# walkernr/neuralMelting

Measured on AMD Instinct MI355X. Metric: MC sweeps/sec (whole node), LJ 4^3 cells, 8x8 PxT grid, higher is better.
Workload: dtype f64

## Files before the change

### include/nm.h

```cpp
#ifndef NM_H
#define NM_H
#include <stdint.h>

#ifdef __cplusplus
extern "C" {
#endif

#define NM_OK 0
#define NM_ERR_ARG (-1)
#define NM_ERR_HIP (-2)
#define NM_ERR_STATE (-3)
#define NM_ERR_UNSUPPORTED (-4)

#define NM_EL_LJ 0
#define NM_EL_AL 1
#define NM_EL_NI 2
#define NM_EL_CU 3

#define NM_THERMO_COLS 17
#define NM_TRACE_COLS 4
#define NM_STATS_COLS 10

typedef struct nm_ctx nm_ctx;

typedef struct nm_config {
    int32_t size;
    int32_t element;
    int32_t natoms;
    int32_t np, nt;
    int32_t row0, nrows;
    int32_t nstps;
    int32_t bulk;
    int32_t iter_revert;
    int32_t device;
    uint32_t seed;
    double ppos, pvol;
// ... 75 lines not shown
```

### neuralmelting_amd/_lib.py

```python
import ctypes as C
import os

_HERE = os.path.dirname(os.path.abspath(__file__))
LIB_PATH = os.environ.get('NM_HIP_LIB') or os.path.join(_HERE, 'libnm_hip.so')

c_double_p = C.POINTER(C.c_double)
c_float_p = C.POINTER(C.c_float)
c_int_p = C.POINTER(C.c_int)
c_uint64_p = C.POINTER(C.c_uint64)
c_int32_p = C.POINTER(C.c_int32)

NM_OK, NM_ERR_ARG, NM_ERR_HIP, NM_ERR_STATE, NM_ERR_UNSUPPORTED = 0, -1, -2, -3, -4
NM_EL_LJ, NM_EL_AL, NM_EL_NI, NM_EL_CU = 0, 1, 2, 3
NM_THERMO_COLS, NM_TRACE_COLS, NM_STATS_COLS = 17, 4, 10

SYMBOLS = ('nm_create', 'nm_destroy', 'nm_last_error', 'nm_create_note', 'nm_nslots', 'nm_natoms', 'nm_cus_per_replica', 'nm_heal_count', 'nm_get_const',
           'nm_get_slots', 'nm_set_slots', 'nm_snapshot', 'nm_snapshot_fetch', 'nm_run_cycles_recorded', 'nm_record_capacity', 'nm_snapshot_pending',
           'nm_set_state', 'nm_get_state', 'nm_init_lattice', 'nm_lattice_state', 'nm_set_thermo', 'nm_set_step', 'nm_run_md', 'nm_run_block', 'nm_run_cycles', 'nm_get_thermo', 'nm_adapt',
           'nm_exchange', 'nm_synchronize', 'nm_get_status', 'nm_format_thrm', 'nm_format_traj', 'nm_append_outputs', 'nm_timing_reset', 'nm_timing_get', 'nm_stats_get', 'nm_eval',
           'nm_set_rng_tape', 'nm_set_exchange_tape', 'nm_set_trace', 'nm_get_trace', 'nm_get_perm', 'nm_set_counters',
           'nm_get_exchange_crit')


DISTR_SYMBOLS = ('nm_distr_histograms', 'nm_distr_angles', 'nm_distr_sfactor', 'nm_distr_bondorder', 'nm_distr_last_error')
PARSE_SYMBOLS = ('nm_parse_thrm', 'nm_parse_traj', 'nm_parse_last_error')


class NMConfig(C.Structure):
    _fields_ = [('size', C.c_int32), ('element', C.c_int32), ('natoms', C.c_int32), ('np', C.c_int32),
# ... 90 lines not shown
```

### neuralmelting_amd/csrc/nm_api.hip

```cpp
#include "../../include/nm.h"
#include "nm_kernels.h"
#include "nm_distr.h"
#include "nm_format.h"
#include "nm_parse.h"
#include "nm_lattice.h"
#include "../../include/nm_distr.h"
#include "../../include/nm_parse.h"

#include <algorithm>
#include <cmath>
#include <cstdio>
#include <cstdlib>
#include <cstring>
#include <deque>
#include <string>
#include <thread>
#include <type_traits>
#include <vector>

using namespace nm;

namespace {

typedef Cfg<512, 4, 256, 192, unsigned char, true, true, 0, 128, true, true> CfgSmallQ2;
// ... 65 lines not shown
static_assert(CfgMidSC::RHO_LDS && CfgMidSCQ4::RHO_LDS && !CfgLargeSC::RHO_LDS, "densities: in LDS at 864 atoms, in the spill at 2048");

thread_local std::string g_create_error;

struct EvPair { hipEvent_t a, b; bool used; uint32_t launch_id; };

}

struct nm_ctx {
    nm_config cfg;
    int N, nslots, slot0, kind;
    int cus;
    bool whole_rows;
    double *d_xbuf;
    uint32_t launch_id;
    double lat, mass, kB, mvv2e, ftm2v, nktv2p, skin, rc;
    int pot;
    double sc_eps, sc_a2, sc_c;
    uint32_t step;
    hipStream_t stream;
    double *d_x, *d_v, *d_box, *d_steps, *d_therm, *d_count, *d_et, *d_pf, *d_tq, *d_stats;
    float *d_ratio;
    int *d_slot2buf, *d_status, *d_status_acc, *d_halt, *d_rerun, *d_nswaps, *d_order;
    unsigned long long *d_last_ticks;
    bool use_order;
    unsigned int *d_census;
    unsigned int census_base = 0, census_cbase = 0;
    unsigned int *d_rowsync = nullptr;
    bool over;
    struct Op { int kind, arg, trace; uint32_t step, launch_id; int rec = -1, rec0 = 0; };
// ... 59 lines not shown
    p.kB = c->kB; p.mvv2e = c->mvv2e; p.ftm2v = c->ftm2v; p.nktv2p = c->nktv2p;
    p.rc = c->rc; p.skin = c->skin;
    p.sc_eps = c->sc_eps; p.sc_a2 = c->sc_a2; p.sc_c = c->sc_c;
    p.x = c->d_x; p.v = c->d_v; p.box = c->d_box; p.steps = c->d_steps; p.therm = c->d_therm;
    p.count = c->d_count; p.ratio = c->d_ratio; p.slot2buf = c->d_slot2buf;
    p.et = c->d_et; p.pf = c->d_pf; p.tq = c->d_tq;
    p.status = c->d_status; p.stats = c->d_stats;
    p.tape = c->d_tape; p.tape_off = c->d_tape_off;
    p.nbr_g = c->d_nbr; p.aux_g = c->d_aux;
    p.prof = c->d_prof;
    p.cus = c->cus; p.xbuf = c->d_xbuf; p.launch_id = c->launch_id;
    p.census = c->cus > 1 ? c->d_census : nullptr; p.over = (c->cus > 1 && c->over) ? 1 : 0;
    p.census_base = c->census_base; p.census_cbase = c->census_cbase;
    p.plain_granules = 1;
    if (const char *e = std::getenv("NM_PLAIN_GRANULES")) p.plain_granules = std::atoi(e);
    p.dbg = 0;
    p.tline = c->d_tline;
    if (const char *e = std::getenv("NM_DBG")) p.dbg = std::atoi(e);
    p.inj_rebuild = -1; p.inj_q = 0;
    const char *e = testing() ? std::getenv("NM_INJECT_OVERFLOW") : nullptr;
    if (e) {
        int n = -1, q = 0;
        if (std::sscanf(e, "%d,%d", &n, &q) >= 1) { p.inj_rebuild = n; p.inj_q = q; }
    }
    p.status_acc = c->d_status_acc; p.halt = c->d_halt; p.rerun_mask = nullptr; p.inj_census = 0;
    p.order = (c->use_order && (c->cus == 1 || c->over)) ? c->d_order : nullptr; p.last_ticks = c->d_last_ticks;
}

unsigned int nm_grid(int nslots, int q) { return q == 1 ? (unsigned int)nslots : (unsigned int)(8 * q * ((nslots + 7) / 8)); }
size_t census_words(int nslots) { return 1 + (size_t)8 * ((nslots + 7) / 8); }
// ... 486 lines not shown

    nm_ctx *c = new nm_ctx();
    c->cfg = *cfg;
    c->h_P.assign(cfg->P, cfg->P + cfg->np); c->h_T.assign(cfg->T, cfg->T + cfg->nt);
    c->cfg.P = c->h_P.data(); c->cfg.T = c->h_T.data();
    c->N = cfg->natoms;
    c->nslots = by_slots ? cfg->nslots : cfg->nrows * cfg->nt;
    c->slot0 = by_slots ? cfg->slot0 : cfg->row0 * cfg->nt;
    c->whole_rows = (c->slot0 % cfg->nt == 0) && (c->nslots % cfg->nt == 0);
    c->cfg.row0 = c->slot0 / cfg->nt;
    c->cfg.nrows = c->whole_rows ? c->nslots / cfg->nt : 0;
    c->step = 0;
    c->trace_on = 0; c->trace_mod = 0; c->trace_cap = 0; c->xtape_n = 0;
    c->ev_next = 0; c->launches = 0; c->total_ms = 0.0;
    c->skin = cfg->natoms <= 512 ? 0.4 : cfg->natoms <= 1024 ? 0.55 : 0.6;
    if (const char *e = std::getenv("NM_SKIN")) { const double v = std::atof(e); if (v > 0.0 && v < 1.0) c->skin = v; }
    c->lat = 1.122; c->mass = 1.0; c->kB = 1.0; c->mvv2e = 1.0; c->ftm2v = 1.0; c->nktv2p = 1.0;
    c->rc = 2.5; c->pot = 0; c->sc_eps = 0.0; c->sc_a2 = 0.0; c->sc_c = 0.0;
    if (const lat::ScElement *s = lat::sc_element(cfg->element)) {
        c->lat = s->lat; c->mass = s->mass; c->kB = 8.617343e-5; c->mvv2e = 1.0364269e-4; c->ftm2v = 1.0 / 1.0364269e-4;
        c->nktv2p = 1.6021765e6; c->rc = s->rc; c->skin = s->skin; c->pot = s->pot;
        c->sc_eps = s->eps; c->sc_a2 = s->a * s->a; c->sc_c = s->c;
        if (cfg->element == NM_EL_AL)
            if (const char *e = std::getenv("NM_SKIN_AL")) { const double v = std::atof(e); if (v > 0.0 && v < 3.0) c->skin = v; }
    }

    c->h_et.resize(c->nslots); c->h_pf.resize(c->nslots); c->h_tq.resize(c->nslots);
    for (int k = 0; k < c->nslots; ++k) {
        const int i = (c->slot0 + k) / cfg->nt, j = (c->slot0 + k) % cfg->nt;
        const double Pi = (double)cfg->P[i], Tj = (double)cfg->T[j];
// ... 1072 lines not shown
```

### neuralmelting_amd/csrc/nm_device.h

```cpp
#pragma once
#include <hip/hip_runtime.h>
#include <stdint.h>

namespace nm {

enum : uint32_t { S_ROLL = 0, S_ACC = 1, S_VOL = 2, S_DISP_XY = 3, S_DISP_Z = 4, S_VEL_A = 5, S_VEL_B = 6,
                  S_EXCH = 7, S_ITER_XY = 8, S_ITER_Z = 9, S_ITER_ACC = 10 };

enum : int { ST_LIST_OVERFLOW = 1, ST_BOX_TOO_SMALL = 2, ST_TAPE_EXHAUSTED = 4, ST_NONFINITE = 8, ST_SYNC_TIMEOUT = 16, ST_NOT_RESIDENT = 32,
             ST_FORCE_RANGE = 64 };

struct KParams {
    int N, nslots, slot0;
    int mod, nstps, bulk, iter_revert;
    int eval_only;
    int md_mode;
    uint32_t seed, step;
    double ppos, pvol, lat, mass;
    double kB, mvv2e, ftm2v, nktv2p;
    double rc, skin;
    double sc_eps, sc_a2, sc_c;
    double *x, *v, *box, *steps, *therm;
    double *count;
    float *ratio;
// ... 19 lines not shown
    unsigned int census_base, census_cbase;
    int *status_acc;
    int *halt;
    const int *rerun_mask;
    int inj_census;
    int over;
    const int *order;
    unsigned long long *last_ticks;
    int ncycles, nt, row0;
    unsigned int *rowbar, *rowgo;
    int *cyc_abort;
    int *nswaps;
    double *xcrit;
    double *rec;
    uint32_t rec_tag0;
};

enum : int { NM_REC_HEAD = 19, NM_REC_BOX = 17, NM_REC_TAG = 18 };

__device__ __forceinline__ void report_status(const KParams &p, int slot, int bits, bool stops)
{
    if (!bits) return;
    atomicOr(&p.status[slot], bits);
    if (p.status_acc) atomicOr(&p.status_acc[slot], bits);
    if (stops && p.halt) atomicCAS(p.halt, 0, (int)p.launch_id);
}
__device__ __forceinline__ bool halted(const KParams &p)
{
    if (!p.halt) return false;
    const int h = __hip_atomic_load(p.halt, __ATOMIC_RELAXED, __HIP_MEMORY_SCOPE_AGENT);
// ... 162 lines not shown
```

### neuralmelting_amd/csrc/nm_kernels.h

```cpp
#pragma once
#include "nm_device.h"
#include "nm_math.h"

namespace nm {

constexpr int NVMAX = 16;

#if defined(NM_PROF) || defined(NM_EXPERIMENT)
#define NM_DBG(bit) (p.dbg & (bit))
#else
#define NM_DBG(bit) false
#endif
#ifdef NM_EXPERIMENT
#define TL_EVALS 512
#define TLINE(k) do { if (tl && tl_n < TL_EVALS && (tid & 63) == 0) tl[((size_t)(q * NW + (tid >> 6)) * TL_EVALS + tl_n) * 8 + (k)] = wall_clock64(); } while (0)
#define TLINE_PREV(k) do { if (tl && tl_n > 0 && tl_n <= TL_EVALS && (tid & 63) == 0) tl[((size_t)(q * NW + (tid >> 6)) * TL_EVALS + tl_n - 1) * 8 + (k)] = wall_clock64(); } while (0)
#ifdef NM_TL_REBUILD
#define RTL(k) do { if (tl && tl_n < TL_EVALS && (tid & 63) == 0) tl[((size_t)(q * NW + (tid >> 6)) * TL_EVALS + tl_n) * 8 + (k)] = wall_clock64(); } while (0)
#undef TLINE
#undef TLINE_PREV
#define TLINE(k) do { if ((k) < 3 && tl && tl_n < TL_EVALS && (tid & 63) == 0) tl[((size_t)(q * NW + (tid >> 6)) * TL_EVALS + tl_n) * 8 + (k)] = wall_clock64(); } while (0)
#define TLINE_PREV(k) do { } while (0)
#else
#define RTL(k) do { } while (0)
#endif
#else
#define TLINE(k) do { } while (0)
#define TLINE_PREV(k) do { } while (0)
#define RTL(k) do { } while (0)
#endif
#ifdef NM_PROF
#define NM_PROF_SLOTS 16
#define PROF_DECL unsigned long long prof_acc[NM_PROF_SLOTS] = {}; unsigned long long prof_t0 = 0;
#define PROF_BEGIN() do { __builtin_amdgcn_sched_barrier(0); prof_t0 = __builtin_readcyclecounter(); __builtin_amdgcn_sched_barrier(0); } while (0)
#define PROF_END(k) do { __builtin_amdgcn_sched_barrier(0); prof_acc[k] += __builtin_readcyclecounter() - prof_t0; __builtin_amdgcn_sched_barrier(0); } while (0)
#else
#define PROF_DECL
#define PROF_BEGIN() do { } while (0)
#define PROF_END(k) do { } while (0)
#endif

extern __shared__ __align__(16) unsigned char nm_lds[];

template <typename T, size_t OFF>
// ... 64 lines not shown
    static constexpr size_t OFF_CNTS = OFF_X0S + (LDS_LIST2 ? A3 : 0);
    static constexpr size_t LDS_NATURAL = OFF_CNTS + (LDS_LIST2 ? pad8((size_t)NMAX * sizeof(unsigned short)) : 0);
    static constexpr size_t LDS_BYTES = LDS_NATURAL > (size_t)82 * 1024 ? LDS_NATURAL : (size_t)82 * 1024;
    static constexpr size_t AUX_SAVES = SAVE_LDS ? (SAVEV_LDS ? 0 : (size_t)3 * NMAX) : (size_t)9 * NMAX + ((size_t)3 * NMAX * 3 + 7) / 8;
    static constexpr bool LIST2 = !LIST_LDS_ || LDS_LIST2_;
    static constexpr size_t AUX_LIST2 = !LIST_LDS_ ? (size_t)3 * NMAX + ((size_t)NMAX + 3) / 4 : 0;
    static constexpr size_t AUX_RHO = (POT_ != 0 && !RHO_LDS) ? (size_t)NMAX : 0;
    static constexpr size_t AUX_DOUBLES = AUX_SAVES + (SAVEF_LDS ? 0 : (size_t)3 * NMAX) + AUX_RHO + AUX_LIST2;
    static constexpr size_t NBR_G_ELEMS = LIST_LDS ? 0 : (size_t)MAXNB * NMAX;
    static constexpr int CH = LIST_LDS ? 1 : 4;
    static_assert(MAXNB % 4 == 0, "MAXNB must be a multiple of the chunk size");
    static constexpr int PW = 8 / (int)sizeof(IdxT);
    static constexpr int LOG2PW = sizeof(IdxT) == 1 ? 3 : 2;
    static_assert(!LIST_LDS || ((sizeof(IdxT) == 1 || sizeof(IdxT) == 2) && MAXNB % (PW * TPA) == 0), "LDS lists: MAXNB a multiple of PW*TPA");
    static constexpr int QMAX = 8;
    static constexpr size_t XBUF_GRANULES = (size_t)4 * NMAX + 4 * QMAX;
    static constexpr size_t XG_PART = (size_t)3 * NMAX, XG_RHO = (size_t)3 * NMAX + 4 * QMAX;
    static constexpr size_t XBUF_DOUBLES = 2 * XBUF_GRANULES;
};

template <class C>
__device__ __attribute__((noinline)) void gaussian_fill(uint32_t tag, int N, int gslot, double mass, uint32_t seed, uint32_t step)
{
    constexpr int BLOCK = C::BLOCK;
    const int tid = threadIdx.x;
    N = __builtin_amdgcn_readfirstlane(N); gslot = __builtin_amdgcn_readfirstlane(gslot);
    tag = __builtin_amdgcn_readfirstlane(tag); seed = __builtin_amdgcn_readfirstlane(seed); step = __builtin_amdgcn_readfirstlane(step);
    mass = uniform(mass);
    double *const gx = (double *)(nm_lds + C::OFF_VEL), *const gy = gx + C::NMAX, *const gz = gy + C::NMAX;
    const double twopi = 6.283185307179586476925286766559;
    const double fac = 1.0 / sqrt(mass);
    for (int w = tid; w < 2 * N; w += BLOCK) {
        const int part = w >= N ? 1 : 0, i = w - part * N;
        uint32_t o[4];
        philox4x32_10((uint32_t)i, part ? S_VEL_B : S_VEL_A, tag, step, seed, (uint32_t)gslot, o);
        const double u1 = u01(o[0], o[1]), u2 = u01(o[2], o[3]);
        const double r = sqrt(-2.0 * log_pos(1.0 - u1));
        double sn, cs;
        sincos_2pi(twopi * u2, sn, cs);
        if (part) gz[i] = r * cs * fac;
        else { gx[i] = r * cs * fac; gy[i] = r * sn * fac; }
    }
}

template <class C>
__device__ __attribute__((noinline)) double velocity_create(double t, uint32_t tag, double L, int N, int gslot, int parity, double mass,
                                                         double mvv2e, double kB, uint32_t seed, uint32_t step, short *im_g)
{
    constexpr int BLOCK = C::BLOCK, NW = C::NW;
    constexpr size_t A1 = (size_t)C::NMAX * sizeof(double);
    const int tid = threadIdx.x;
    LdsArr<double, C::OFF_POS> px; LdsArr<double, C::OFF_POS + A1> py; LdsArr<double, C::OFF_POS + 2 * A1> pz;
    LdsArr<double, C::OFF_VEL> vx; LdsArr<double, C::OFF_VEL + A1> vy; LdsArr<double, C::OFF_VEL + 2 * A1> vz;
    LdsArr<double, C::OFF_RED> red;
    typename ArrSel<C::SAVE_LDS, short, C::OFF_IMG>::type im;
    if constexpr (!C::SAVE_LDS) {
        const unsigned long long b = (unsigned long long)(uintptr_t)im_g;
// ... 85 lines not shown
    typename ArrSel<C::SAVEF_LDS, double, C::OFF_SAVF + 2 * A1>::type sfz;
    typename ArrSel<C::SAVE_LDS, double, C::OFF_X0>::type x0; typename ArrSel<C::SAVE_LDS, double, C::OFF_X0 + A1>::type y0;
    typename ArrSel<C::SAVE_LDS, double, C::OFF_X0 + 2 * A1>::type z0;
    typename ArrSel<C::SAVE_LDS, short, C::OFF_IMG>::type im;
    typename ArrSel<C::SAVE_LDS, signed char, C::OFF_WN>::type wn;
    LdsArr<unsigned short, C::OFF_CNT> cnt;
    typename ArrSel<C::LIST_LDS, IdxT, C::OFF_NBR>::type nbr;
    LdsArr<double, C::OFF_RED> red;
    typename ArrSel<C::RHO_LDS || !C::EAM, double, C::OFF_RHO>::type rho;
    int parity = 0;
    double L = 0.0, L0 = 0.0, U = 0.0, W = 0.0;
    double bc_L = -1.0, bc_L0 = -1.0, bc_invL = 0.0, bc_sc = 0.0, bc_thr2 = 0.0;
    bool bc_bad = true;
    double psum[4] = { 0.0, 0.0, 0.0, 0.0 };
    __device__ __forceinline__ double &ust(int k) const { return ((double *)(nm_lds + C::OFF_UST))[(tid >> 6) * C::UST_PER_WAVE + k]; }
    enum : int { F_LIST_OK = 1, F_FRESH = 2, F_SAVED_FRESH = 4, F_LIST_SAVED = 8, F_REBUILT = 16 };
    int flags = 0;
    __device__ __forceinline__ bool fresh() const { return (flags & F_FRESH) != 0; }
    __device__ __forceinline__ void set_fresh(bool b) { flags = b ? (flags | F_FRESH) : (flags & ~F_FRESH); }
    int status = 0;
    typename ArrSel<C::LDS_LIST2, double, C::OFF_X0S>::type x0s; typename ArrSel<C::LDS_LIST2, double, C::OFF_X0S + A1>::type y0s;
    typename ArrSel<C::LDS_LIST2, double, C::OFF_X0S + 2 * A1>::type z0s;
    typename ArrSel<C::LDS_LIST2, unsigned short, C::OFF_CNTS>::type cnts;
    double L0s = 0.0;
    int list_cur = 0;
    __device__ __forceinline__ IdxT *nbr_cur() const
    {
        if constexpr (C::LDS_LIST2) return (IdxT *)(nm_lds + C::OFF_NBR + (size_t)list_cur * C::LIST_BYTES);
        else return nbr.ptr();
    }
    bool same_xcd = false;
    const double *tape = nullptr;
    int tpos = 0, tlen = 0;
    double st_evals = 0.0, st_rebuilds = 0.0, st_eevals = 0.0, st_pairs = 0.0;
// ... 113 lines not shown
            if (x < 0.0) x = 0.0;
        }
        return d;
    }
    __device__ void wrap()
    {
        for (int i = tid; i < N; i += BLOCK) {
            im[3 * i] = (short)(im[3 * i] + wrap1(px[i]));
            im[3 * i + 1] = (short)(im[3 * i + 1] + wrap1(py[i]));
            im[3 * i + 2] = (short)(im[3 * i + 2] + wrap1(pz[i]));
        }
    }
    __device__ void save(bool with_v)
    {
        if (with_v && Q > 1) {
            for (int i = tid; i < N; i += BLOCK)
                if (i < a0 || i >= a1) { sx[i] = px[i]; sy[i] = py[i]; sz[i] = pz[i]; svx[i] = vx[i]; svy[i] = vy[i]; svz[i] = vz[i]; }
            NM_FOR_OWN(i) { sx[i] = px[i]; sy[i] = py[i]; sz[i] = pz[i]; svx[i] = vx[i]; svy[i] = vy[i]; svz[i] = vz[i]; }
        } else
        for (int i = tid; i < N; i += BLOCK) {
            sx[i] = px[i]; sy[i] = py[i]; sz[i] = pz[i];
            if (with_v) { svx[i] = vx[i]; svy[i] = vy[i]; svz[i] = vz[i]; }
        }
        flags &= ~(F_LIST_SAVED | F_REBUILT);
        if (C::LIST2 && (flags & F_LIST_OK)) flags |= F_LIST_SAVED;
        flags = fresh() ? (flags | F_SAVED_FRESH) : (flags & ~F_SAVED_FRESH);
        if (fresh())
            NM_FOR_OWN(i) { sfx[i] = fx[i]; sfy[i] = fy[i]; sfz[i] = fz[i]; }
    }
    __device__ void restore(bool with_v)
// ... 747 lines not shown
        for (int u = 0; u < W; ++u) rn[u] = sc_rep(rm[u], q2[u], a1r * y[u]);
#pragma unroll
        for (int u = 0; u < W; ++u) {
            const double dF = 0.5 * cc * (isi + rj[u]);
            fp[u] = eps * ((double)C::SC_N * rn[u] - 6.0 * dF * rm[u]) * t[u];
        }
#pragma unroll
        for (int u = 0; u < W; ++u) {
            ax += dx[u] * fp[u]; ay += dy[u] * fp[u]; az += dz[u] * fp[u];
            if (WANT_E) { e += eps * rn[u]; w += r2[u] * fp[u]; np += in[u] ? 1.0 : 0.0; }
        }
    }

    typedef unsigned long long u64x2 __attribute__((ext_vector_type(2)));
    static constexpr unsigned long long POISON = 0x5555555555555554ull;
    __device__ __forceinline__ unsigned long long magic() const
    {
        return ((unsigned long long)p.launch_id << 32 | (unsigned long long)(uint32_t)(gen + 1)) * 0x9E3779B97F4A7C15ull | 1ull;
    }
    __device__ __forceinline__ void put_granule(double *g, double v, unsigned long long mg)
    {
        u64x2 w;
        w.x = (unsigned long long)__double_as_longlong(v);
        w.y = w.x ^ mg;
        if (same_xcd) asm volatile("global_store_dwordx4 %0, %1, off\n\ts_nop 1" ::"v"(g), "v"(w) : "memory");
        else asm volatile("global_store_dwordx4 %0, %1, off sc1\n\ts_nop 1" ::"v"(g), "v"(w) : "memory");
    }
    template <int K>
    __device__ __forceinline__ bool get_granules(double *const (&g)[K], unsigned long long mg, double (&out)[K], int &timeout, int &poisoned)
    {
        unsigned long long t0 = 0;
        int spins = 0;
        for (;;) {
            u64x2 w[K];
// ... 27 lines not shown
                return true;
            }
            static constexpr int POLL_SLEEP = 1;
            __builtin_amdgcn_s_sleep(POLL_SLEEP);
            if ((++spins & 63) == 0) {
                const unsigned long long now = wall_clock64();
                if (t0 == 0) t0 = now | 1ull;
                else if (now - t0 > 200000000ull) { timeout = 1; return false; }
            }
        }
    }

    __device__ __forceinline__ unsigned long long my_magic() const { return magic() ^ ((status & ST_LIST_OVERFLOW) ? POISON : 0ull); }

    template <int K>
    __device__ void exchange_sums(double (&s)[K])
    {
        static_assert(K == 4, "one instantiation: callers pad with zeros");
        if (Q == 1) return;
        double *xg = xb + (size_t)(gen & 1) * C::XBUF_DOUBLES;
        const unsigned long long mg = magic();
        if (tid < K) {
            double mine = s[0];
#pragma unroll
            for (int k = 1; k < K; ++k) mine = (tid == k) ? s[k] : mine;
            put_granule(xg + 2 * (size_t)(C::XG_PART + 4 * q + tid), mine, my_magic());
        }
        int timeout = 0, poisoned = 0;
        const int lane = tid & 63;
        double v[K];
#pragma unroll
        for (int k = 0; k < K; ++k) v[k] = 0.0;
        if (lane < Q) {
            double *gs[K];
#pragma unroll
            for (int k = 0; k < K; ++k) gs[k] = xg + 2 * (C::XG_PART + 4 * lane + k);
            get_granules<K>(gs, mg, v, timeout, poisoned);
        }
        double t[K];
#pragma unroll
        for (int k = 0; k < K; ++k) {
            t[k] = 0.0;
// ... 40 lines not shown
    {
        check_atom(c, x, y, z, x0[i], y0[i], z0[i]);
    }
    __device__ __forceinline__ void check_atom(ListCheck &c, double x, double y, double z, double rx, double ry, double rz) const
    {
        double dx = x - c.sc * rx, dy = y - c.sc * ry, dz = z - c.sc * rz;
        dx -= L * rint(dx * c.invL); dy -= L * rint(dy * c.invL); dz -= L * rint(dz * c.invL);
        if (dx * dx + dy * dy + dz * dz > c.thr2) c.bad = 1;
    }

    __device__ bool advance_and_share(int mode, double dtfm, double h)
    {
        int timeout = 0, poisoned = 0;
        double *xg = xb ? xb + (size_t)(gen & 1) * C::XBUF_DOUBLES : nullptr;
        const unsigned long long mg = magic(), mgp = my_magic();
        NM_FOR_OWN(i) {
            const double gx = fx[i], gy = fy[i], gz = fz[i];
            if (mode == 3) { px[i] = gx; py[i] = gy; pz[i] = gz; continue; }
            double ux = __builtin_fma(dtfm, gx, vx[i]), uy = __builtin_fma(dtfm, gy, vy[i]), uz = __builtin_fma(dtfm, gz, vz[i]);
            if (mode == 2) { ux = __builtin_fma(dtfm, gx, ux); uy = __builtin_fma(dtfm, gy, uy); uz = __builtin_fma(dtfm, gz, uz); }
            vx[i] = ux; vy[i] = uy; vz[i] = uz;
            const double nx = __builtin_fma(h, ux, px[i]), ny = __builtin_fma(h, uy, py[i]), nz = __builtin_fma(h, uz, pz[i]);
            px[i] = nx; py[i] = ny; pz[i] = nz;
            if (Q > 1) {
                put_granule(xg + 2 * (size_t)i, nx, mgp);
                put_granule(xg + 2 * (size_t)(NMAX + i), ny, mgp);
                put_granule(xg + 2 * (size_t)(2 * NMAX + i), nz, mgp);
            }
        }
        ListCheck c;
        check_begin(c);
        NM_FOR_OWN(i) check_atom(c, i, px[i], py[i], pz[i]);
        if (Q > 1) {
            const int nown = a1 - a0, nother = N - nown;
            const int shift = ((nown + 63) & ~63) % BLOCK;
            for (int o = (tid + BLOCK - shift) % BLOCK; o < nother; o += BLOCK) {
                const int i = o < a0 ? o : o + nown;
                double *const g3[3] = { xg + 2 * (size_t)i, xg + 2 * (size_t)(NMAX + i), xg + 2 * (size_t)(2 * NMAX + i) };
                double x3[3];
                const double rx = x0[i], ry = y0[i], rz = z0[i];
                if (get_granules<3>(g3, mg, x3, timeout, poisoned)) {
                    px[i] = x3[0]; py[i] = x3[1]; pz[i] = x3[2];
                    check_atom(c, x3[0], x3[1], x3[2], rx, ry, rz);
                }
            }
            ++gen;
        }
        set_fresh(false);
        TLINE_PREV(6);
        const int fl = block_any3<NW, NVMAX>(timeout != 0, poisoned != 0, c.bad != 0, red, parity);
        TLINE_PREV(7);
        if (fl & 1) status |= ST_SYNC_TIMEOUT;
        if (fl & 2) status |= ST_LIST_OVERFLOW;
        return (fl & 4) != 0;
    }

    __device__ void eval(bool have_need = false, bool pre_need = false, bool final_kick = false, double dtfm = 0.0)
    {
        if (status & (ST_SYNC_TIMEOUT | ST_LIST_OVERFLOW)) return;
        if (!(L >= 2.0 * p.rc)) { status |= ST_BOX_TOO_SMALL; __syncthreads(); return; }
        bool need = !(flags & F_LIST_OK);
// ... 66 lines not shown
        set_fresh(true);
    }

    __device__ void take_sums()
    {
        U = 0.5 * psum[0]; W = 0.5 * psum[1];
        if constexpr (C::HALF)
            if (psum[2] >= FR_TAG) {
                fr_hit = 1; set_fresh(false);
                psum[2] = fmod(psum[2], FR_TAG);
            }
        st_eevals += 1.0; st_pairs += 0.5 * psum[2];
        if (!(U == U) || isinf(U)) status |= ST_NONFINITE;
    }
    int layout_pad = -1;
    __device__ double finish_sums(double extra)
    {
        double s[4] = { psum[0], psum[1], psum[2], extra };
        exchange_sums<4>(s);
        psum[0] = s[0]; psum[1] = s[1]; psum[2] = s[2];
        take_sums();
        return s[3];
    }

    __device__ __forceinline__ double hmc_velocities(double t, uint32_t tag)
    {
        short *img = nullptr;
        if constexpr (!C::SAVE_LDS) img = im.g;
        const double mv2 = velocity_create<C>(t, tag, L, N, gslot, parity, p.mass, p.mvv2e, p.kB, p.seed, p.step, img);
        parity ^= 1;
        return uniform(mv2);
    }

    __device__ void delta_single(int k, double ox, double oy, double oz, double nx, double ny, double nz, double &dE, double &dW)
    {
        box_consts();
        const double invL = bc_invL, rc2 = p.rc * p.rc;
        double s[2] = { 0.0, 0.0 };
        for (int j = tid; j < N; j += BLOCK) {
            const double xj = px[j], yj = py[j], zj = pz[j];
            double ax = nx - xj, ay = ny - yj, az = nz - zj, bx = ox - xj, by = oy - yj, bz = oz - zj;
            ax -= L * rint(ax * invL); ay -= L * rint(ay * invL); az -= L * rint(az * invL);
            bx -= L * rint(bx * invL); by -= L * rint(by * invL); bz -= L * rint(bz * invL);
            const double ra = ax * ax + ay * ay + az * az, rb = bx * bx + by * by + bz * bz;
// ... 620 lines not shown
#endif
    R.load(buf);
    R.L = uniform(p.eval_only ? p.box[buf] : q6(p.box[buf]));
    R.wrap();

    double &et = R.ust(0), &pf = R.ust(1), &t = R.ust(2), &dx = R.ust(3), &dv = R.ust(4), &dt = R.ust(5);
    double &ntp = R.ust(6), &nap = R.ust(7), &ntv = R.ust(8), &nav = R.ust(9), &nth = R.ust(10), &nah = R.ust(11);
    double &U0 = R.ust(12), &W0 = R.ust(13), &c_pe = R.ust(14), &c_vol = R.ust(15), &c_volnew = R.ust(16), &c_boxl = R.ust(17);
    et = p.et[slot]; pf = p.pf[slot]; t = p.tq[slot];
    dx = p.steps[3 * buf]; dv = p.steps[3 * buf + 1]; dt = p.steps[3 * buf + 2];
    ntp = p.count[6 * slot]; nap = p.count[6 * slot + 1]; ntv = p.count[6 * slot + 2];
    nav = p.count[6 * slot + 3]; nth = p.count[6 * slot + 4]; nah = p.count[6 * slot + 5];
    U0 = 0.0; W0 = 0.0; c_pe = 0.0; c_vol = 0.0; c_volnew = 0.0; c_boxl = 0.0;
    double &nth_entry = R.ust(22);
    nth_entry = nth;
    const int fatal = ST_BOX_TOO_SMALL | ST_LIST_OVERFLOW | ST_SYNC_TIMEOUT | ST_FORCE_RANGE;

    int phase = PH_INIT, m = 0;
    bool skip_eval = false;
    double &mv2new = R.ust(18);
    mv2new = 0.0;
    bool have_need = false, pre_need = false;
    double &c_h = R.ust(19), &c_dtfm = R.ust(20), &mv2_0 = R.ust(21);
    c_h = 0.0; c_dtfm = 0.0; mv2_0 = 0.0;

    for (;;) {
        const int st_before = R.status;
        if (!skip_eval) {
            R.eval(have_need, pre_need, phase == PH_HMC_STEP, c_dtfm);
            if (!(st_before & fatal) && !(R.status & (ST_BOX_TOO_SMALL | ST_SYNC_TIMEOUT)))
                mv2new = R.finish_sums(phase == PH_HMC_STEP ? R.psum[3] : 0.0);
        }
        skip_eval = false;
        have_need = false;
        if (R.status & fatal) {
            if (R.Q > 1 && (R.status & ST_LIST_OVERFLOW)) R.publish_poison();
            break;
        }
#ifdef NM_PROF
        unsigned long long &prof_t0 = R.prof_t0; unsigned long long (&prof_acc)[NM_PROF_SLOTS] = R.prof_acc;
        const int prof_phase = phase;
#endif
        PROF_BEGIN();

        bool move_done = false, acc = false;
        double crit = 0.0, branch = 0.0;
// ... 27 lines not shown
            branch = 0.0; move_done = true;
        } else if (phase == PH_VMC) {
            const double penew = R.U / et;
            crit = (penew - c_pe) + pf * (c_volnew - c_vol) - (double)(N + 1) * log(c_volnew / c_vol);
            acc = R.metropolis(crit, S_ACC, (uint32_t)m, 0);
            if (acc) nav += 1.0;
            else { R.L = uniform(q6(c_boxl)); R.restore(false); R.wrap(); R.U = U0; R.W = W0; }
            branch = 1.0; move_done = true;
        } else if (phase == PH_HMC_START) {
            R.save(true);
            U0 = R.U; W0 = R.W;
            c_pe = R.U / et + 0.5 * p.mvv2e * mv2_0 / et;
            PROF_END(5 + prof_phase);
            const double dtfm_ = uniform(c_dtfm), h_ = uniform(c_h);
            PROF_BEGIN();
            pre_need = R.advance_and_share(1, dtfm_, h_);
            PROF_END(9);
            const int nfo = p.nstps - 1;
            for (int s = 0; s < nfo; ++s) {
                if (__builtin_amdgcn_readfirstlane(R.status) & fatal) break;
                R.eval_force(pre_need, dtfm_, h_);
                if (__builtin_amdgcn_readfirstlane(R.status) & fatal) break;
                PROF_BEGIN();
                pre_need = R.advance_and_share(C::HALF ? 2 : 3, dtfm_, h_);
                PROF_END(9);
            }
            have_need = true;
            phase = PH_HMC_STEP;
            continue;
        } else {
            const double etotnew = R.U / et + 0.5 * p.mvv2e * mv2new / et;
            crit = etotnew - c_pe;
            bool out_of_range = false;
            if constexpr (C::HALF) out_of_range = R.fr_hit != 0;
            if (out_of_range) crit = __builtin_huge_val();
            if (!PLAIN && p.md_mode) {
                acc = true;
                if (out_of_range) R.status |= ST_FORCE_RANGE;
            } else {
                acc = R.metropolis(crit, S_ACC, (uint32_t)m, 0) && !out_of_range;
                if (acc) nah += 1.0;
                else { R.restore(true); R.wrap(); R.U = U0; R.W = W0; }
            }
            branch = 2.0; move_done = true;
        }
        if (move_done) {
            if constexpr (!PLAIN)
                if (p.trace && writer) {
                    double *tr = p.trace + ((size_t)slot * p.mod + m) * 4;
                    tr[0] = branch; tr[1] = acc ? 1.0 : 0.0; tr[2] = crit; tr[3] = R.U;
                }
            ++m;
        }

        PROF_END(5 + prof_phase);
        bool pending = false;
        while (m < p.mod && !pending) {
            PROF_BEGIN();
            const double roll = (!PLAIN && p.md_mode) ? 2.0 : R.draw_scalar(S_ROLL, (uint32_t)m, 0);
            if (roll <= p.ppos && (PLAIN || p.bulk)) {
                ntp += 1.0;
// ... 5 lines not shown
                    uint32_t o[4], q[4];
                    philox4x32_10((uint32_t)i, S_DISP_XY, tag, p.step, p.seed, (uint32_t)R.gslot, o);
                    philox4x32_10((uint32_t)i, S_DISP_Z, tag, p.step, p.seed, (uint32_t)R.gslot, q);
                    R.px[i] += a * 2.0 * (u01(o[0], o[1]) - 0.5);
                    R.py[i] += a * 2.0 * (u01(o[2], o[3]) - 0.5);
                    R.pz[i] += a * 2.0 * (u01(q[0], q[1]) - 0.5);
                }
                R.set_fresh(false);
                R.wrap();
                phase = PH_BULK; pending = true;
                PROF_END(10);
            } else if (!PLAIN && roll <= p.ppos) {
                if constexpr (!PLAIN) {
                    double c2 = 0.0;
                    const int na = R.iter_pmc((uint32_t)m, et, dx, ntp, nap, c2);
                    if (__builtin_amdgcn_readfirstlane(R.status) & fatal) break;
                    if constexpr (C::EAM) {
                        c_vol = (double)na; c_volnew = c2;
                        phase = PH_ITER_END; pending = true;
                    } else {
                        if (p.trace && writer) {
                            double *tr = p.trace + ((size_t)slot * p.mod + m) * 4;
                            tr[0] = 3.0; tr[1] = (double)na; tr[2] = c2; tr[3] = R.U;
                        }
                        ++m;
                    }
                    PROF_END(13);
                }
            } else if (roll <= p.ppos + p.pvol) {
                ntv += 1.0;
// ... 65 lines not shown
        p.box[buf] = R.L;
        double *c = p.count + 6 * (size_t)slot;
        c[0] = ntp; c[1] = nap; c[2] = ntv; c[3] = nav; c[4] = nth; c[5] = nah;
        float *r = p.ratio + 3 * (size_t)slot;
        r[0] = (ntp > 0.0) ? (float)nap / (float)ntp : 0.0f;
        r[1] = (ntv > 0.0) ? (float)nav / (float)ntv : 0.0f;
        r[2] = (nth > 0.0) ? (float)nah / (float)nth : 0.0f;
        if constexpr (!PLAIN)
            if (R.tape && R.tpos > R.tlen) R.status |= ST_TAPE_EXHAUSTED;
        report_status(p, slot, R.status, false);
        double *st = p.stats + NM_STATS_COLS * (size_t)slot;
        st[0] += R.st_evals; st[1] += R.st_rebuilds; st[2] += R.st_eevals; st[3] += R.st_pairs;
        const unsigned long long ticks = wall_clock64() - t_entry;
        if (p.last_ticks) p.last_ticks[slot] = ticks;
        st[4] += (double)ticks; st[5] += R.same_xcd ? 1.0 : 0.0; st[6] += 1.0; st[7] += nth - nth_entry; st[9] = (double)C::MAXNB;
#ifdef NM_PROF
        if (p.prof) for (int q = 0; q < NM_PROF_SLOTS; ++q) p.prof[(size_t)slot * NM_PROF_SLOTS + q] += R.prof_acc[q];
#endif
    }
    return 0;
}

template <class C, bool PLAIN = false>
__global__ void __launch_bounds__(C::BLOCK) nm_block_kernel(const KParams p)
{
    (void)nm_block_body<C, true, PLAIN>(p);
}

__global__ void nm_order_kernel(int nslots, const unsigned long long *ticks, int *order)
{
// ... 252 lines not shown
```

Measured before the change: 1.485 million.

## Publish forces on board so HMC start advances remote atoms locally

When a replica is split across several blocks, each block now publishes its own atoms' forces to a global board at the end of the preceding evaluation. At the first HMC half-step, every block then recomputes the other blocks' positions locally from those forces and its own saved velocities, instead of waiting for a cross-block position exchange. The board is read during velocity creation so the load overlaps other work, with a timeout fallback. This costs extra global writes per evaluation and a larger exchange buffer, and it is only active for configs with LDS-saved forces and partial lists (LOCAL_START), unless disabled through NM_START_HANDOVER.

```diff
diff --git a/include/nm.h b/include/nm.h
--- a/include/nm.h
+++ b/include/nm.h
@@ -19,7 +19,7 @@
 
 #define NM_THERMO_COLS 17
 #define NM_TRACE_COLS 4
-#define NM_STATS_COLS 10
+#define NM_STATS_COLS 11
 
 typedef struct nm_ctx nm_ctx;
 
diff --git a/neuralmelting_amd/_lib.py b/neuralmelting_amd/_lib.py
--- a/neuralmelting_amd/_lib.py
+++ b/neuralmelting_amd/_lib.py
@@ -12,7 +12,7 @@
 
 NM_OK, NM_ERR_ARG, NM_ERR_HIP, NM_ERR_STATE, NM_ERR_UNSUPPORTED = 0, -1, -2, -3, -4
 NM_EL_LJ, NM_EL_AL, NM_EL_NI, NM_EL_CU = 0, 1, 2, 3
-NM_THERMO_COLS, NM_TRACE_COLS, NM_STATS_COLS = 17, 4, 10
+NM_THERMO_COLS, NM_TRACE_COLS, NM_STATS_COLS = 17, 4, 11
 
 SYMBOLS = ('nm_create', 'nm_destroy', 'nm_last_error', 'nm_create_note', 'nm_nslots', 'nm_natoms', 'nm_cus_per_replica', 'nm_heal_count', 'nm_get_const',
            'nm_get_slots', 'nm_set_slots', 'nm_snapshot', 'nm_snapshot_fetch', 'nm_run_cycles_recorded', 'nm_record_capacity', 'nm_snapshot_pending',
diff --git a/neuralmelting_amd/csrc/nm_api.hip b/neuralmelting_amd/csrc/nm_api.hip
--- a/neuralmelting_amd/csrc/nm_api.hip
+++ b/neuralmelting_amd/csrc/nm_api.hip
@@ -103,6 +103,7 @@
     bool whole_rows;
     double *d_xbuf;
     uint32_t launch_id;
+    int start_handover = 0;
     double lat, mass, kB, mvv2e, ftm2v, nktv2p, skin, rc;
     int pot;
     double sc_eps, sc_a2, sc_c;
@@ -192,6 +193,7 @@
     p.census_base = c->census_base; p.census_cbase = c->census_cbase;
     p.plain_granules = 1;
     if (const char *e = std::getenv("NM_PLAIN_GRANULES")) p.plain_granules = std::atoi(e);
+    p.start_handover = c->start_handover;
     p.dbg = 0;
     p.tline = c->d_tline;
     if (const char *e = std::getenv("NM_DBG")) p.dbg = std::atoi(e);
@@ -708,6 +710,7 @@
     c->trace_on = 0; c->trace_mod = 0; c->trace_cap = 0; c->xtape_n = 0;
     c->ev_next = 0; c->launches = 0; c->total_ms = 0.0;
     c->skin = cfg->natoms <= 512 ? 0.4 : cfg->natoms <= 1024 ? 0.55 : 0.6;
+    if (const char *e = std::getenv("NM_START_HANDOVER")) c->start_handover = std::atoi(e) != 0;
     if (const char *e = std::getenv("NM_SKIN")) { const double v = std::atof(e); if (v > 0.0 && v < 1.0) c->skin = v; }
     c->lat = 1.122; c->mass = 1.0; c->kB = 1.0; c->mvv2e = 1.0; c->ftm2v = 1.0; c->nktv2p = 1.0;
     c->rc = 2.5; c->pot = 0; c->sc_eps = 0.0; c->sc_a2 = 0.0; c->sc_c = 0.0;
diff --git a/neuralmelting_amd/csrc/nm_device.h b/neuralmelting_amd/csrc/nm_device.h
--- a/neuralmelting_amd/csrc/nm_device.h
+++ b/neuralmelting_amd/csrc/nm_device.h
@@ -57,6 +57,7 @@
     double *xcrit;
     double *rec;
     uint32_t rec_tag0;
+    int start_handover;
 };
 
 enum : int { NM_REC_HEAD = 19, NM_REC_BOX = 17, NM_REC_TAG = 18 };
diff --git a/neuralmelting_amd/csrc/nm_kernels.h b/neuralmelting_amd/csrc/nm_kernels.h
--- a/neuralmelting_amd/csrc/nm_kernels.h
+++ b/neuralmelting_amd/csrc/nm_kernels.h
@@ -24,10 +24,16 @@
 #else
 #define RTL(k) do { } while (0)
 #endif
+#if defined(NM_TL_START) && !defined(NM_TL_REBUILD)
+#define TLINE_START() TLINE_PREV(5)
+#else
+#define TLINE_START() do { } while (0)
+#endif
 #else
 #define TLINE(k) do { } while (0)
 #define TLINE_PREV(k) do { } while (0)
 #define RTL(k) do { } while (0)
+#define TLINE_START() do { } while (0)
 #endif
 #ifdef NM_PROF
 #define NM_PROF_SLOTS 16
@@ -122,8 +128,11 @@
     static constexpr int LOG2PW = sizeof(IdxT) == 1 ? 3 : 2;
     static_assert(!LIST_LDS || ((sizeof(IdxT) == 1 || sizeof(IdxT) == 2) && MAXNB % (PW * TPA) == 0), "LDS lists: MAXNB a multiple of PW*TPA");
     static constexpr int QMAX = 8;
-    static constexpr size_t XBUF_GRANULES = (size_t)4 * NMAX + 4 * QMAX;
+    static constexpr bool LOCAL_START = SAVEF_LDS && NLIST_ < NMAX_;
+    static constexpr int UST_BOARD = 24, UST_BOARD_MAGIC = 25, UST_BOARD_OWN = 26, UST_BOARD_LATE = 28;
+    static constexpr size_t XBUF_GRANULES = (size_t)(LOCAL_START ? 7 : 4) * NMAX + 4 * QMAX;
     static constexpr size_t XG_PART = (size_t)3 * NMAX, XG_RHO = (size_t)3 * NMAX + 4 * QMAX;
+    static constexpr size_t XG_BOARD = (size_t)4 * NMAX + 4 * QMAX;
     static constexpr size_t XBUF_DOUBLES = 2 * XBUF_GRANULES;
 };
 
@@ -138,6 +147,30 @@
     double *const gx = (double *)(nm_lds + C::OFF_VEL), *const gy = gx + C::NMAX, *const gz = gy + C::NMAX;
     const double twopi = 6.283185307179586476925286766559;
     const double fac = 1.0 / sqrt(mass);
+    [[maybe_unused]] unsigned long long bw[6] = { 0, 0, 0, 0, 0, 0 }, bmg = 0;
+    [[maybe_unused]] const unsigned long long *bg = nullptr;
+    [[maybe_unused]] unsigned long long *us = nullptr;
+    [[maybe_unused]] int bi = -1;
+    if constexpr (C::LOCAL_START) {
+        static_assert(C::NMAX <= C::BLOCK, "one atom per thread");
+        us = (unsigned long long *)(nm_lds + C::OFF_UST) + (tid >> 6) * C::UST_PER_WAVE;
+        const unsigned long long b = us[C::UST_BOARD];
+        bg = (const unsigned long long *)(uintptr_t)(((unsigned long long)(uint32_t)__builtin_amdgcn_readfirstlane((uint32_t)(b >> 32)) << 32) |
+                                                     (unsigned long long)(uint32_t)__builtin_amdgcn_readfirstlane((uint32_t)b));
+        if (bg) {
+            bmg = us[C::UST_BOARD_MAGIC];
+            const int a0 = (int)(us[C::UST_BOARD_OWN] & 0xffffu), a1 = (int)(us[C::UST_BOARD_OWN] >> 16), nown = a1 - a0;
+            if (tid < N - nown) {
+                bi = tid < a0 ? tid : tid + nown;
+                bg += 2 * (size_t)bi;
+#pragma unroll
+                for (int c = 0; c < 3; ++c) {
+                    bw[2 * c] = __hip_atomic_load(bg + 2 * (size_t)c * C::NMAX, __ATOMIC_RELAXED, __HIP_MEMORY_SCOPE_AGENT);
+                    bw[2 * c + 1] = __hip_atomic_load(bg + 2 * (size_t)c * C::NMAX + 1, __ATOMIC_RELAXED, __HIP_MEMORY_SCOPE_AGENT);
+                }
+            }
+        }
+    }
     for (int w = tid; w < 2 * N; w += BLOCK) {
         const int part = w >= N ? 1 : 0, i = w - part * N;
         uint32_t o[4];
@@ -149,6 +182,31 @@
         if (part) gz[i] = r * cs * fac;
         else { gx[i] = r * cs * fac; gy[i] = r * sn * fac; }
     }
+    if constexpr (C::LOCAL_START)
+        if (bg) {
+            int late = 0;
+            if (bi >= 0) {
+                unsigned long long t0 = 0;
+                int spins = 0;
+                while (((bw[0] ^ bw[1]) != bmg) | ((bw[2] ^ bw[3]) != bmg) | ((bw[4] ^ bw[5]) != bmg)) {
+                    __builtin_amdgcn_s_sleep(1);
+                    if ((++spins & 63) == 0) {
+                        const unsigned long long now = wall_clock64();
+                        if (t0 == 0) t0 = now | 1ull;
+                        else if (now - t0 > 200000000ull) { late = 1; break; }
+                    }
+#pragma unroll
+                    for (int c = 0; c < 3; ++c) {
+                        bw[2 * c] = __hip_atomic_load(bg + 2 * (size_t)c * C::NMAX, __ATOMIC_RELAXED, __HIP_MEMORY_SCOPE_AGENT);
+                        bw[2 * c + 1] = __hip_atomic_load(bg + 2 * (size_t)c * C::NMAX + 1, __ATOMIC_RELAXED, __HIP_MEMORY_SCOPE_AGENT);
+                    }
+                }
+                double *const sf = (double *)(nm_lds + C::OFF_SAVF);
+#pragma unroll
+                for (int c = 0; c < 3; ++c) sf[(size_t)c * C::NMAX + bi] = __longlong_as_double((long long)bw[2 * c]);
+            }
+            if (__ballot(late) != 0) us[C::UST_BOARD_LATE] = 1;
+        }
 }
 
 template <class C>
@@ -264,10 +322,11 @@
     bool bc_bad = true;
     double psum[4] = { 0.0, 0.0, 0.0, 0.0 };
     __device__ __forceinline__ double &ust(int k) const { return ((double *)(nm_lds + C::OFF_UST))[(tid >> 6) * C::UST_PER_WAVE + k]; }
-    enum : int { F_LIST_OK = 1, F_FRESH = 2, F_SAVED_FRESH = 4, F_LIST_SAVED = 8, F_REBUILT = 16 };
+    __device__ __forceinline__ unsigned long long &ustu(int k) const { return ((unsigned long long *)(nm_lds + C::OFF_UST))[(tid >> 6) * C::UST_PER_WAVE + k]; }
+    enum : int { F_LIST_OK = 1, F_FRESH = 2, F_SAVED_FRESH = 4, F_LIST_SAVED = 8, F_REBUILT = 16, F_BOARD = 32, F_SF_ALL = 64 };
     int flags = 0;
     __device__ __forceinline__ bool fresh() const { return (flags & F_FRESH) != 0; }
-    __device__ __forceinline__ void set_fresh(bool b) { flags = b ? (flags | F_FRESH) : (flags & ~F_FRESH); }
+    __device__ __forceinline__ void set_fresh(bool b) { flags = b ? (flags | F_FRESH) : (flags & ~(C::LOCAL_START ? F_FRESH | F_BOARD : F_FRESH)); }
     int status = 0;
     typename ArrSel<C::LDS_LIST2, double, C::OFF_X0S>::type x0s; typename ArrSel<C::LDS_LIST2, double, C::OFF_X0S + A1>::type y0s;
     typename ArrSel<C::LDS_LIST2, double, C::OFF_X0S + 2 * A1>::type z0s;
@@ -411,6 +470,13 @@
     __device__ void save(bool with_v)
     {
         if (with_v && Q > 1) {
+            if constexpr (C::LOCAL_START) {
+                const int nown = a1 - a0, shift = ((nown + 63) & ~63) % BLOCK;
+                for (int o = (tid + BLOCK - shift) % BLOCK; o < N - nown; o += BLOCK) {
+                    const int i = o < a0 ? o : o + nown;
+                    sx[i] = px[i]; sy[i] = py[i]; sz[i] = pz[i]; svx[i] = vx[i]; svy[i] = vy[i]; svz[i] = vz[i];
+                }
+            } else
             for (int i = tid; i < N; i += BLOCK)
                 if (i < a0 || i >= a1) { sx[i] = px[i]; sy[i] = py[i]; sz[i] = pz[i]; svx[i] = vx[i]; svy[i] = vy[i]; svz[i] = vz[i]; }
             NM_FOR_OWN(i) { sx[i] = px[i]; sy[i] = py[i]; sz[i] = pz[i]; svx[i] = vx[i]; svy[i] = vy[i]; svz[i] = vz[i]; }
@@ -1188,10 +1254,11 @@
 
     typedef unsigned long long u64x2 __attribute__((ext_vector_type(2)));
     static constexpr unsigned long long POISON = 0x5555555555555554ull;
-    __device__ __forceinline__ unsigned long long magic() const
-    {
-        return ((unsigned long long)p.launch_id << 32 | (unsigned long long)(uint32_t)(gen + 1)) * 0x9E3779B97F4A7C15ull | 1ull;
-    }
+    __device__ __forceinline__ unsigned long long magic_at(int g) const
+    {
+        return ((unsigned long long)p.launch_id << 32 | (unsigned long long)(uint32_t)(g + 1)) * 0x9E3779B97F4A7C15ull | 1ull;
+    }
+    __device__ __forceinline__ unsigned long long magic() const { return magic_at(gen); }
     __device__ __forceinline__ void put_granule(double *g, double v, unsigned long long mg)
     {
         u64x2 w;
@@ -1249,7 +1316,7 @@
     __device__ __forceinline__ unsigned long long my_magic() const { return magic() ^ ((status & ST_LIST_OVERFLOW) ? POISON : 0ull); }
 
     template <int K>
-    __device__ void exchange_sums(double (&s)[K])
+    __device__ void exchange_sums(double (&s)[K], bool board = false)
     {
         static_assert(K == 4, "one instantiation: callers pad with zeros");
         if (Q == 1) return;
@@ -1261,6 +1328,15 @@
             for (int k = 1; k < K; ++k) mine = (tid == k) ? s[k] : mine;
             put_granule(xg + 2 * (size_t)(C::XG_PART + 4 * q + tid), mine, my_magic());
         }
+        if constexpr (C::LOCAL_START)
+            if (board) {
+                const unsigned long long mgp = my_magic();
+                NM_FOR_OWN(i) {
+                    put_granule(xg + 2 * (C::XG_BOARD + (size_t)i), fx[i], mgp);
+                    put_granule(xg + 2 * (C::XG_BOARD + (size_t)(NMAX + i)), fy[i], mgp);
+                    put_granule(xg + 2 * (C::XG_BOARD + (size_t)(2 * NMAX + i)), fz[i], mgp);
+                }
+            }
         int timeout = 0, poisoned = 0;
         const int lane = tid & 63;
         double v[K];
@@ -1331,6 +1407,8 @@
         int timeout = 0, poisoned = 0;
         double *xg = xb ? xb + (size_t)(gen & 1) * C::XBUF_DOUBLES : nullptr;
         const unsigned long long mg = magic(), mgp = my_magic();
+        const bool local = C::LOCAL_START && mode >= 4;
+        if (mode == 1 || local) TLINE_START();
         NM_FOR_OWN(i) {
             const double gx = fx[i], gy = fy[i], gz = fz[i];
             if (mode == 3) { px[i] = gx; py[i] = gy; pz[i] = gz; continue; }
@@ -1339,7 +1417,7 @@
             vx[i] = ux; vy[i] = uy; vz[i] = uz;
             const double nx = __builtin_fma(h, ux, px[i]), ny = __builtin_fma(h, uy, py[i]), nz = __builtin_fma(h, uz, pz[i]);
             px[i] = nx; py[i] = ny; pz[i] = nz;
-            if (Q > 1) {
+            if (Q > 1 && !local) {
                 put_granule(xg + 2 * (size_t)i, nx, mgp);
                 put_granule(xg + 2 * (size_t)(NMAX + i), ny, mgp);
                 put_granule(xg + 2 * (size_t)(2 * NMAX + i), nz, mgp);
@@ -1351,17 +1429,33 @@
         if (Q > 1) {
             const int nown = a1 - a0, nother = N - nown;
             const int shift = ((nown + 63) & ~63) % BLOCK;
+            double *const gr = local ? xb + (size_t)((gen - 1) & 1) * C::XBUF_DOUBLES + 2 * C::XG_BOARD : xg;
+            const unsigned long long mgr = local ? magic_at(gen - 1) : mg;
+            if constexpr (C::LOCAL_START)
+                if (local && ustu(C::UST_BOARD_LATE) != 0) timeout = 1;
             for (int o = (tid + BLOCK - shift) % BLOCK; o < nother; o += BLOCK) {
                 const int i = o < a0 ? o : o + nown;
-                double *const g3[3] = { xg + 2 * (size_t)i, xg + 2 * (size_t)(NMAX + i), xg + 2 * (size_t)(2 * NMAX + i) };
+                double *const g3[3] = { gr + 2 * (size_t)i, gr + 2 * (size_t)(NMAX + i), gr + 2 * (size_t)(2 * NMAX + i) };
                 double x3[3];
                 const double rx = x0[i], ry = y0[i], rz = z0[i];
-                if (get_granules<3>(g3, mg, x3, timeout, poisoned)) {
+                bool got = true;
+                if constexpr (C::LOCAL_START) {
+                    if (mode == 5) { x3[0] = sfx[i]; x3[1] = sfy[i]; x3[2] = sfz[i]; }
+                    else got = get_granules<3>(g3, mgr, x3, timeout, poisoned);
+                    if (local && got) {
+                        if (mode == 4) { sfx[i] = x3[0]; sfy[i] = x3[1]; sfz[i] = x3[2]; }
+                        x3[0] = __builtin_fma(h, __builtin_fma(dtfm, x3[0], vx[i]), px[i]);
+                        x3[1] = __builtin_fma(h, __builtin_fma(dtfm, x3[1], vy[i]), py[i]);
+                        x3[2] = __builtin_fma(h, __builtin_fma(dtfm, x3[2], vz[i]), pz[i]);
+                    }
+                } else got = get_granules<3>(g3, mg, x3, timeout, poisoned);
+                if (got) {
                     px[i] = x3[0]; py[i] = x3[1]; pz[i] = x3[2];
                     check_atom(c, x3[0], x3[1], x3[2], rx, ry, rz);
                 }
             }
-            ++gen;
+            if (local) flags |= F_SF_ALL;
+            else ++gen;
         }
         set_fresh(false);
         TLINE_PREV(6);
@@ -1458,12 +1552,14 @@
         if (!(U == U) || isinf(U)) status |= ST_NONFINITE;
     }
     int layout_pad = -1;
-    __device__ double finish_sums(double extra)
+    __device__ double finish_sums(double extra, bool board = false)
     {
         double s[4] = { psum[0], psum[1], psum[2], extra };
-        exchange_sums<4>(s);
+        exchange_sums<4>(s, board);
         psum[0] = s[0]; psum[1] = s[1]; psum[2] = s[2];
         take_sums();
+        if constexpr (C::LOCAL_START)
+            if (board && Q > 1) flags |= F_BOARD;
         return s[3];
     }
 
@@ -1471,7 +1567,16 @@
     {
         short *img = nullptr;
         if constexpr (!C::SAVE_LDS) img = im.g;
+        [[maybe_unused]] bool pre = false;
+        if constexpr (C::LOCAL_START) {
+            pre = Q > 1 && (flags & F_BOARD);
+            ustu(C::UST_BOARD) = pre ? (unsigned long long)(uintptr_t)(xb + (size_t)((gen - 1) & 1) * C::XBUF_DOUBLES + 2 * C::XG_BOARD) : 0ull;
+            ustu(C::UST_BOARD_MAGIC) = magic_at(gen - 1);
+            ustu(C::UST_BOARD_OWN) = (unsigned long long)a0 | (unsigned long long)a1 << 16;
+        }
         const double mv2 = velocity_create<C>(t, tag, L, N, gslot, parity, p.mass, p.mvv2e, p.kB, p.seed, p.step, img);
+        if constexpr (C::LOCAL_START)
+            if (pre) flags = (flags & ~F_BOARD) | F_SF_ALL;
         parity ^= 1;
         return uniform(mv2);
     }
@@ -2122,6 +2227,10 @@
     U0 = 0.0; W0 = 0.0; c_pe = 0.0; c_vol = 0.0; c_volnew = 0.0; c_boxl = 0.0;
     double &nth_entry = R.ust(22);
     nth_entry = nth;
+    if constexpr (C::LOCAL_START) {
+        R.ust(23) = 0.0;
+        R.ustu(C::UST_BOARD_LATE) = 0;
+    }
     const int fatal = ST_BOX_TOO_SMALL | ST_LIST_OVERFLOW | ST_SYNC_TIMEOUT | ST_FORCE_RANGE;
 
     int phase = PH_INIT, m = 0;
@@ -2137,7 +2246,12 @@
         if (!skip_eval) {
             R.eval(have_need, pre_need, phase == PH_HMC_STEP, c_dtfm);
             if (!(st_before & fatal) && !(R.status & (ST_BOX_TOO_SMALL | ST_SYNC_TIMEOUT)))
-                mv2new = R.finish_sums(phase == PH_HMC_STEP ? R.psum[3] : 0.0);
+            {
+                bool board = false;
+                if constexpr (C::LOCAL_START)
+                    board = !p.start_handover && !p.eval_only && ((phase == PH_INIT || phase == PH_HMC_START) ? m : m + 1) < p.mod;
+                mv2new = R.finish_sums(phase == PH_HMC_STEP ? R.psum[3] : 0.0, board);
+            }
         }
         skip_eval = false;
         have_need = false;
@@ -2195,7 +2309,13 @@
             PROF_END(5 + prof_phase);
             const double dtfm_ = uniform(c_dtfm), h_ = uniform(c_h);
             PROF_BEGIN();
-            pre_need = R.advance_and_share(1, dtfm_, h_);
+            int smode = 1;
+            if constexpr (C::LOCAL_START)
+                if (R.Q > 1 && !p.start_handover && (R.flags & (R.F_BOARD | R.F_SF_ALL))) {
+                    smode = (R.flags & R.F_BOARD) ? 4 : 5;
+                    R.ust(23) += 1.0;
+                }
+            pre_need = R.advance_and_share(smode, dtfm_, h_);
             PROF_END(9);
             const int nfo = p.nstps - 1;
             for (int s = 0; s < nfo; ++s) {
@@ -2226,6 +2346,8 @@
             branch = 2.0; move_done = true;
         }
         if (move_done) {
+            if constexpr (C::LOCAL_START)
+                if (acc) R.flags &= ~R.F_SF_ALL;
             if constexpr (!PLAIN)
                 if (p.trace && writer) {
                     double *tr = p.trace + ((size_t)slot * p.mod + m) * 4;
@@ -2261,6 +2383,7 @@
                 if constexpr (!PLAIN) {
                     double c2 = 0.0;
                     const int na = R.iter_pmc((uint32_t)m, et, dx, ntp, nap, c2);
+                    if constexpr (C::LOCAL_START) R.flags &= ~R.F_SF_ALL;
                     if (__builtin_amdgcn_readfirstlane(R.status) & fatal) break;
                     if constexpr (C::EAM) {
                         c_vol = (double)na; c_volnew = c2;
@@ -2356,6 +2479,7 @@
         const unsigned long long ticks = wall_clock64() - t_entry;
         if (p.last_ticks) p.last_ticks[slot] = ticks;
         st[4] += (double)ticks; st[5] += R.same_xcd ? 1.0 : 0.0; st[6] += 1.0; st[7] += nth - nth_entry; st[9] = (double)C::MAXNB;
+        if constexpr (C::LOCAL_START) st[10] += R.ust(23);
 #ifdef NM_PROF
         if (p.prof) for (int q = 0; q < NM_PROF_SLOTS; ++q) p.prof[(size_t)slot * NM_PROF_SLOTS + q] += R.prof_acc[q];
 #endif
```

Result: faster. 1.510 million (median of 6 runs) (+1.7%).
